# mxngjxa/lshrs

Measured on AMD Instinct MI355X. Metric: vectors/sec hashed (768-d, num_perm=256), higher is better.
Workload: dtype bf16x3 on the matrix cores + f32 replay of the host BLAS inside the proven window (bit-exact f32 sign result)

## Files before the change

### lshrs_amd/csrc/lshrs_common.h

```cpp
#ifndef LSHRS_COMMON_H
#define LSHRS_COMMON_H

#include <hip/hip_runtime.h>
#include <hip/hip_ext.h>
#include <stdint.h>
#include <stddef.h>
#include <math.h>
#include <type_traits>

#include "lshrs_hip.h"

typedef float f32x4 __attribute__((ext_vector_type(4)));
typedef float f32x16 __attribute__((ext_vector_type(16)));
typedef uint32_t u32x2 __attribute__((ext_vector_type(2)));
typedef uint32_t u32x4 __attribute__((ext_vector_type(4)));
typedef __bf16 bf16x8 __attribute__((ext_vector_type(8)));
typedef __bf16 bf16x2 __attribute__((ext_vector_type(2)));
typedef uint16_t u16x8 __attribute__((ext_vector_type(8)));

#define GLOBAL_AS __attribute__((address_space(1)))
#define LDS_AS __attribute__((address_space(3)))
#define LSHRS_HIDDEN __attribute__((visibility("hidden")))

namespace lshrs {
// ... 64 lines not shown
  w.wa = p; w.wb = p + wc; w.wt = p + 2 * wc;
  w.wamax = p + 3 * wc; w.wbmax = w.wamax + cbp; w.wtmax = w.wbmax + cbp; w.wtmax_fine = w.wtmax + cbp;
  return w;
}
struct SigCompact { bool on; int bpb; int ncb; };
inline SigCompact sig_compact(const SigGeom& g, int num_bands, int rows) {
  SigCompact c{false, 0, 0};
  if (g.nt != 8 || rows > 128) return c;
  c.bpb = 256 / rows;
  c.ncb = (num_bands + c.bpb - 1) / c.bpb;
  c.on = c.ncb < g.cb;
  return c;
}
inline int64_t sig_pad4(int64_t v) { return (v + 3) & ~(int64_t)3; }
struct SigCompactWs { float *image, *norms, *norm_max, *wa, *wb, *wamax, *wbmax; int *padcol, *bytetab; };
inline int64_t sig_compact_floats(const SigGeom& g, const SigCompact& c) {
  if (!c.on) return 0;
  return (int64_t)c.ncb * g.ktiles * 8192 + 3 * (int64_t)c.ncb * 256 + 3 * sig_pad4(c.ncb) + (int64_t)c.ncb * 256 * 3;
}
struct SigResident { bool on; int nct; int kt; };
inline SigResident sig_resident(int num_bands, int rows, int dim) {
  SigResident r{false, 0, 0};
  const int64_t real = (int64_t)num_bands * rows;
  if (real > 256 || dim > 256 || dim < 8) return r;
  r.nct = (((int)real + 15) / 16 + 3) / 4 * 4;
  r.kt = dim <= 64 ? 2 : (dim <= 128 ? 4 : 8);
  r.on = r.nct * r.kt <= 64;
  return r;
}
__host__ __device__ inline int res_colmap(int nct, int ct, int m) {
  const int g = m >> 2, e = m & 3, k = ct >> 3;
  const int bits = 4 * (nct - 8 * k < 8 ? nct - 8 * k : 8);
  return 128 * k + bits * g + (bits - 1) - (4 * (ct & 7) + e);
}
inline int64_t sig_resident_floats(const SigResident& r) {
  return r.on ? (int64_t)r.kt * 8192 + 3 * 256 + 3 * 4 + 256 * 3 : 0;
}
inline int64_t sig_workspace_floats(const SigGeom& g, int num_bands, int rows, int dim) {
  return sig_window_offset_floats(g) + sig_window_floats(g) + sig_compact_floats(g, sig_compact(g, num_bands, rows)) +
         sig_resident_floats(sig_resident(num_bands, rows, dim));
}
inline SigCompactWs sig_compact_ws(float* base, const SigGeom& g, const SigCompact& c) {
  SigCompactWs w;
  float* p = base + sig_window_offset_floats(g) + sig_window_floats(g);
  w.image = p; p += (int64_t)c.ncb * g.ktiles * 8192;
  w.norms = p; p += (int64_t)c.ncb * 256;
  w.norm_max = p; p += sig_pad4(c.ncb);
  w.wa = p; p += (int64_t)c.ncb * 256;
  w.wb = p; p += (int64_t)c.ncb * 256;
  w.wamax = p; p += sig_pad4(c.ncb);
  w.wbmax = p; p += sig_pad4(c.ncb);
  w.padcol = reinterpret_cast<int*>(p); p += (int64_t)c.ncb * 256;
  w.bytetab = reinterpret_cast<int*>(p);
  return w;
}
inline SigCompactWs sig_resident_ws(float* base, const SigGeom& g, int num_bands, int rows, const SigResident& r) {
  SigCompactWs w;
  float* p = base + sig_window_offset_floats(g) + sig_window_floats(g) + sig_compact_floats(g, sig_compact(g, num_bands, rows));
  w.image = p; p += (int64_t)r.kt * 8192;
  w.norms = p; p += 256;
  w.norm_max = p; p += 4;
  w.wa = p; p += 256;
  w.wb = p; p += 256;
  w.wamax = p; p += 4;
  w.wbmax = p; p += 4;
  w.padcol = reinterpret_cast<int*>(p); p += 256;
// ... 103 lines not shown
  const float w1 = rem == 1 ? 0.f : (rem == 2 ? v[3] : v[2]);
  const float w2 = rem == 3 ? v[3] : 0.f;
  f32x4 r = part ? f32x4{w0, w1, w2, 0.f} : v;
#pragma unroll
  for (int e = 0; e < 4; ++e) r[e] = gone ? 0.f : r[e];
  return r;
}

__device__ __forceinline__ float row_lanes_sum(const float& v) {
  float s = v + __shfl_xor(v, 16);
  s += __shfl_xor(s, 32);
  return s;
}
__device__ __forceinline__ float row_lanes_max(const float& v) {
  float m = __builtin_fmaxf(v, __shfl_xor(v, 16));
  m = __builtin_fmaxf(m, __shfl_xor(m, 32));
  return m;
}

template <bool RAW_ROOT>
__device__ __forceinline__ float window_root(float v) { return RAW_ROOT ? __builtin_amdgcn_sqrtf(v) : sqrtf(v); }
template <bool RAW_ROOT>
__device__ __forceinline__ float window_hi(float s2, float am, float tau) {
  float window = window_root<RAW_ROOT>(s2) * tau * 1.001f;
  if (am != 0.f && !(am >= 0x1p-32f && am <= 0x1p32f)) window = __builtin_inff();
  return window;
}
template <bool RAW_ROOT>
__device__ __forceinline__ float window_mid(float m2, float tau_b) {
  const float wb = window_root<RAW_ROOT>(m2) * tau_b * 1.001f;
  return wb < __builtin_inff() ? wb : 0.f;
}

constexpr int kEntryColBits = 21;
__host__ __device__ __forceinline__ int64_t flag_entry(int64_t row, int col) { return (row << kEntryColBits) | (int64_t)col; }
__host__ __device__ __forceinline__ int64_t entry_row(int64_t entry) { return entry >> kEntryColBits; }
__host__ __device__ __forceinline__ int entry_col(int64_t entry) { return (int)(entry & ((1 << kEntryColBits) - 1)); }

__device__ __forceinline__ float ykeep(const float& window, const float& y) { return window < __builtin_inff() ? y : __builtin_nanf(""); }

template <bool ALIGNBIT>
__device__ __forceinline__ uint32_t key_byte(uint32_t lo, uint32_t hi, int src, uint32_t mask) {
  const uint32_t v = ALIGNBIT ? __builtin_amdgcn_alignbit(hi, lo, (uint32_t)(src & 31)) : (uint32_t)((((uint64_t)hi << 32) | lo) >> (src & 31));
  return v & mask;
}

struct FixArgs {
  const float* X;
  int64_t ldx;
  int dim;
  int ktiles;
  const float* prow;
  const float* norms;
  const float* tie_coef;
  uint8_t* keys;
  int row_bytes;
  int padcols;
  const int64_t* flag_list;
  const int* flag_count;
  int flag_cap;
  int64_t row_base;
  int64_t* tie_list;
  int tie_cap;
  int* tie_count;
  float tau;
  int blas_model;
// ... 162 lines not shown
```

### lshrs_amd/csrc/sig16.hip

```cpp
#include "lshrs_common.h"

using namespace lshrs;

namespace {
#ifndef LSHRS_X_AUX
#define LSHRS_X_AUX 0
#endif
template <bool COMPACT, bool PARTIAL = false, int W = 8>
__global__ __launch_bounds__(64 * W, 8 / W) void sig16_kernel(const SigArgs args) {
  constexpr int RT = 2;
  constexpr int kRows = 32 * W;
  constexpr int kXDepth = W == 8 ? 3 : 2;
  constexpr int kS1ListCap = W == 8 ? 8192 : 4096;
  constexpr int kWaveRows = 16 * RT;
  constexpr int kPP = 16 / W;
  constexpr int kXPS = RT;
  constexpr int kE = 6 * RT;
  constexpr int kSlices = 12 * RT;
  constexpr int kPHalf = 16 * kFragFloats;
  constexpr int kXTile = kRows * kKTile;
  constexpr int kXWave = kWaveRows * kKTile;
  constexpr int kRingFloats = 3 * kPHalf + kXDepth * kXTile;
  constexpr int kIssues = (kPP + kXPS) / 2;
  constexpr int kIssueStep = kE / kIssues;
  static_assert((kPP + kXPS) % 2 == 0 && kE % kIssues == 0, "DMA issue slots");
  static_assert(3 * kS1ListCap <= kRingFloats, "the epilogue's list stage reuses the ring");
  constexpr int kTabOff = 3 * kS1ListCap;
  constexpr int kWndOff = W == 8 ? kRingFloats : kTabOff + 768 + kRows * 8;
  static_assert(kWndOff + 2 * kRows + 4 <= (W == 8 ? kRingFloats + 512 + 4 : kRingFloats), "windows and counters");
  __shared__ __attribute__((aligned(16))) float lds[W == 8 ? kRingFloats + 512 + 4 : kRingFloats];
  struct Bf16Pairs { bf16x2 p[4]; };

  const int tid = threadIdx.x;
  const int lane = tid & 63;
  const int wave = __builtin_amdgcn_readfirstlane(tid >> 6);
  const int r16 = lane & 15, g = lane >> 4;
  const int ncb = args.ncb;
  const int bid = blockIdx.x;
  const int cb = (bid >> 3) % ncb;
  const int row_tile = ((bid >> 3) / ncb) * 8 + (bid & 7);
  int au_slot = -1, au_rw = -1, au_lane = 0, au_q = 0;
  if (args.audit_list != nullptr) {
    const unsigned u = (unsigned)bid * (unsigned)W + (unsigned)wave;
    if ((int)(u % (unsigned)args.audit_div) == args.audit_phase) {
      const unsigned h = audit_hash(u, args.audit_seed);
      au_slot = (int)(u / (unsigned)args.audit_div);
      au_rw = (int)(h & 15u);
      au_q = (int)((h >> 4) & 7u);
      au_lane = (int)((h >> 7) & 63u);
    }
  }
  if ((int64_t)row_tile * kRows >= args.n) {
    if (au_slot >= 0 && lane == 0) args.audit_list[au_slot] = -1;
    return;
  }
  const int ktiles = args.ktiles;
  const int stages = 2 * ktiles, lasts = stages - 1;
  const char* img = reinterpret_cast<const char*>(args.image) + (size_t)cb * ktiles * 32768;
  const int64_t blk_row0 = (int64_t)row_tile * kRows;
  const int64_t row0 = blk_row0 + wave * kWaveRows;
  const char* xblk = reinterpret_cast<const char*>(args.X + blk_row0 * args.ldx);

  unsigned xfo[2 * RT], xrd[2];
// ... 92 lines not shown
    const int pair = q / 3, step = q % 3, rt = pair >> 2, pr = pair & 3, c = pr >> 1, e = 2 * (pr & 1);
    const float v0 = xr[rt][c][e], v1 = xr[rt][c][e + 1];
    if (step == 0) {
      bf16x2 hp;
      asm("v_cvt_pk_bf16_f32 %0, %1, %2" : "=v"(hp) : "v"(v0), "v"(v1));
      hi[rt].p[pr] = hp;
      r0 = v0 - (float)hp[0];
      r1 = v1 - (float)hp[1];
    } else if (step == 1) {
      bf16x2 mp;
      asm("v_cvt_pk_bf16_f32 %0, %1, %2" : "=v"(mp) : "v"(r0), "v"(r1));
      mid[rt].p[pr] = mp;
    } else {
      ss[rt] = __builtin_amdgcn_fdot2_f32_bf16(hi[rt].p[pr], hi[rt].p[pr], ss[rt], false);
#ifndef LSHRS_AB_NO_XMID_NORM
      sm[rt] = __builtin_amdgcn_fdot2_f32_bf16(mid[rt].p[pr], mid[rt].p[pr], sm[rt], false);
#endif
      asm("v_max3_f32 %0, |%1|, |%2|, %0" : "+v"(amax[rt]) : "v"(v0), "v"(v1));
    }
  };
  auto read_eighth = [&](unsigned base, int e, f32x4 (&f)[2][2]) {
#pragma unroll
    for (int j = 0; j < 2; ++j) {
      f[j][0] = *reinterpret_cast<const LDS_AS f32x4*>(lds_b + (base + (unsigned)(((2 * e + j) * 2 + 0) * 1024)));
      f[j][1] = *reinterpret_cast<const LDS_AS f32x4*>(lds_b + (base + (unsigned)(((2 * e + j) * 2 + 1) * 1024)));
    }
  };
  const unsigned lane16 = (unsigned)lane * 16u;
  auto mfma_one = [&](int ct0, int k, const f32x4 (&f)[2][2], const Bf16Pairs (&hi)[RT], const Bf16Pairs (&mid)[RT], const bool drain = false) {
    const int term = k / (2 * RT), j = (k / RT) % 2, rt = k % RT;
    const bf16x8 a = __builtin_bit_cast(bf16x8, term == 2 ? mid[rt] : hi[rt]);
    const bf16x8 b = __builtin_bit_cast(bf16x8, f[j][term == 1 ? 1 : 0]);
#ifdef LSHRS_T16_BUILTIN
    acc[rt][ct0 + j] = __builtin_amdgcn_mfma_f32_16x16x32_bf16(a, b, acc[rt][ct0 + j], 0, 0, 0);
#else
    if (drain) asm volatile("v_mfma_f32_16x16x32_bf16 %0, %1, %2, %0\n\ts_nop 7\n\ts_nop 4" : "+a"(acc[rt][ct0 + j]) : "v"(a), "v"(b));
    else asm volatile("v_mfma_f32_16x16x32_bf16 %0, %1, %2, %0" : "+a"(acc[rt][ct0 + j]) : "v"(a), "v"(b));
#endif
  };

  f32x4 fa[2][2], fb[2][2];
  Bf16Pairs hs0[RT], ms0[RT], hs1[RT], ms1[RT];

  auto stage = [&](int s, const int ch, const bool first, const Bf16Pairs (&hc)[RT], const Bf16Pairs (&mc)[RT],
                   const Bf16Pairs (&hp)[RT], const Bf16Pairs (&mp)[RT], Bf16Pairs (&hn)[RT], Bf16Pairs (&mn)[RT]) {
    unsigned st = lane16 + fr0;
    asm volatile("" : "+v"(st));
    read_eighth(st, 0, fa);
    __builtin_amdgcn_sched_barrier(0);
#pragma unroll
    for (int k = 0; k < kE; ++k) {
      if (!first) mfma_one(8 * (1 - ch) + 6, k, fb, hp, mp);
      if (ch == 0) {
        if (k % 3 != 2) split_step(2 * kSlices / 3 + (k / 3) * 2 + k % 3, hn, mn);
      }
      __builtin_amdgcn_sched_barrier(0);
    }
    __builtin_amdgcn_s_waitcnt(0xC07F);
    __builtin_amdgcn_sched_barrier(0);
    wait_vmcnt<kXPS>();
    read_eighth(st, 1, fb);
    if (ch == 1) read_x((s >> 1) + 1, xq1);
    __builtin_amdgcn_sched_barrier(0);
#pragma unroll
    for (int k = 0; k < kE; ++k) {
      mfma_one(8 * ch + 0, k, fa, hc, mc);
      __builtin_amdgcn_sched_barrier(0);
    }
    __builtin_amdgcn_s_waitcnt(0xC07F);
    __builtin_amdgcn_sched_barrier(0);
// ... 33 lines not shown
  };
  auto tile = [&](int t, const bool first, Bf16Pairs (&hc)[RT], Bf16Pairs (&mc)[RT], Bf16Pairs (&hp)[RT], Bf16Pairs (&mp)[RT]) {
    stage(2 * t, 0, first, hc, mc, hp, mp, hc, mc);
    stage(2 * t + 1, 1, false, hc, mc, hc, mc, hp, mp);
  };

  auto issue_prologue = [&]() {
    const int t1 = ktiles > 1 ? 1 : 0;
#pragma unroll
    for (int d = 0; d < kPP; ++d) issue_frag(d, 0, fr0);
#pragma unroll
    for (int d = 0; d < kXPS; ++d) { issue_x(d, 0, xq0); issue_x(kXPS + d, 0, xq0); }
#pragma unroll
    for (int d = 0; d < kPP; ++d) issue_frag(d, 1, fr1);
#pragma unroll
    for (int d = 0; d < kXPS; ++d) { issue_x(d, t1, xq1); issue_x(kXPS + d, t1, xq1); }
  };
#ifndef LSHRS_AB_NO_STATIC_PRIO
  if (W == 8 && wave >= 4) __builtin_amdgcn_s_setprio(1);
#endif
  issue_prologue();
  zero_tile_state();
  wait_vmcnt<kPP + 2 * kXPS>();
  __builtin_amdgcn_s_barrier();
  read_x(0, xq0);
#pragma unroll
  for (int q = 0; q < 2 * kSlices / 3; ++q) split_step(q, hs0, ms0);
  tile(0, true, hs0, ms0, hs1, ms1);
  int t = 1;
  for (; t + 1 < ktiles; t += 2) {
    tile(t, false, hs1, ms1, hs0, ms0);
    tile(t + 1, false, hs0, ms0, hs1, ms1);
  }
  if (t < ktiles) {
    tile(t, false, hs1, ms1, hs0, ms0);
#pragma unroll
    for (int k = 0; k < kE; ++k) mfma_one(14, k, fb, hs1, ms1, true);
  } else {
#pragma unroll
    for (int k = 0; k < kE; ++k) mfma_one(14, k, fb, hs0, ms0, true);
  }
  asm volatile("s_waitcnt vmcnt(0)" ::: "memory");
  __builtin_amdgcn_s_barrier();
  asm volatile("s_nop 7\n\ts_nop 7\n\ts_nop 7" ::: "memory");
#pragma unroll
  for (int rt = 0; rt < RT; ++rt)
#pragma unroll
    for (int ct = 0; ct < 16; ++ct) asm volatile("" : "+a"(acc[rt][ct]));

  if (args.clock_probe != nullptr && tid == 0) {
    const unsigned long long slot = (unsigned long long)blockIdx.x;
    args.clock_probe[2 * slot] = __builtin_amdgcn_s_memtime() - t_shader;
    args.clock_probe[2 * slot + 1] = __builtin_amdgcn_s_memrealtime() - t_real;
  }

  int r16e = r16, ge = g, lanee = lane;
  asm volatile("" : "+v"(r16e), "+v"(ge), "+v"(lanee));
  int64_t* l_list = reinterpret_cast<int64_t*>(lds);
  float* l_y = lds + 2 * kS1ListCap;
  int* l_count = reinterpret_cast<int*>(lds + kWndOff + 2 * kRows);
  if (tid == 0) l_count[0] = 0;

  float* wnd_lds = lds + kWndOff + wave * kWaveRows;
  float* wnb_lds = lds + kWndOff + kRows + wave * kWaveRows;
  float* coef_lds = lds + kTabOff;
  static_assert(kTabOff + 512 <= kRingFloats, "coefficients behind the list stage");
#pragma unroll
  for (int i = tid; i < 512; i += 64 * W) coef_lds[i] = i < 256 ? args.wa[cb * 256 + i] : args.wb[cb * 256 + i - 256];
  int* padcol_lds = reinterpret_cast<int*>(lds + kTabOff + 512);
  uint32_t* cw_lds = reinterpret_cast<uint32_t*>(lds + kTabOff + 768);
  static_assert(kTabOff + 768 + kRows * 8 <= kRingFloats, "compact tables behind the coefficients");
  if (COMPACT && tid < 256) padcol_lds[tid] = args.padcol[cb * 256 + tid];
#pragma unroll
  for (int rt = 0; rt < RT; ++rt) {
    const float s2 = row_lanes_sum(ss[rt]), m2 = row_lanes_sum(sm[rt]), am = row_lanes_max(amax[rt]);
    const int64_t myrow = row0 + 16 * rt + r16e;
    if (ge == 0) {
      wnd_lds[16 * rt + r16e] = window_hi<false>(s2, am, args.tau);
      wnb_lds[16 * rt + r16e] = window_mid<false>(m2, args.tau_b);
      if (cb == 0 && args.row_flags != nullptr && myrow < args.n) args.row_flags[myrow] = row_flag_byte(am, s2);
    }
  }
  __builtin_amdgcn_s_waitcnt(0xC07F);
  __builtin_amdgcn_s_barrier();

  const float amax_cb = args.wamax[cb], bmax_cb = args.wbmax[cb];
  {
    uint32_t A[2] = {0u, 0u}, B[2] = {0u, 0u};
#pragma unroll
    for (int rt = 0; rt < 2; ++rt) {
      const f32x4 wnd = *reinterpret_cast<const f32x4*>(wnd_lds + 16 * rt + 4 * ge);
      const f32x4 wnb = *reinterpret_cast<const f32x4*>(wnb_lds + 16 * rt + 4 * ge);
      float tsmax = __builtin_fmaxf(__builtin_fmaxf(wnd[0], wnd[1]), __builtin_fmaxf(wnd[2], wnd[3]));
      if (!(wnd[0] < __builtin_inff()) || !(wnd[1] < __builtin_inff()) || !(wnd[2] < __builtin_inff()) ||
          !(wnd[3] < __builtin_inff()))
        tsmax = __builtin_inff();
      tsmax = tsmax * amax_cb +
              __builtin_fmaxf(__builtin_fmaxf(wnb[0], wnb[1]), __builtin_fmaxf(wnb[2], wnb[3])) * bmax_cb;
      tsmax = tsmax > 0.f ? tsmax : -1.f;
#pragma unroll
      for (int w = 0; w < 8; ++w) {
        float m = __builtin_inff();
#pragma unroll
        for (int reg = 0; reg < 4; ++reg) {
          const float y0 = acc[rt][2 * w][reg], y1 = acc[rt][2 * w + 1][reg];
          const int p0 = 8 * rt + reg * 2;
#ifdef LSHRS_AB_CHEAP_SIGNS
          A[w & 1] = __builtin_amdgcn_alignbit(A[w & 1], __float_as_uint(y0), 31u);
          B[w & 1] = __builtin_amdgcn_alignbit(B[w & 1], __float_as_uint(y1), 31u);
#else
          deposit_positive(A[w & 1], y0, 4 * p0 + (w >> 1), 4 * (p0 + 1) + (w >> 1));
          deposit_positive(B[w & 1], y1, 4 * p0 + (w >> 1), 4 * (p0 + 1) + (w >> 1));
#endif
          asm("v_min3_f32 %0, |%1|, |%2|, %0" : "+v"(m) : "v"(y0), "v"(y1));
        }
        const bool aud = au_rw == 8 * rt + w;
        if (__builtin_amdgcn_ballot_w64(!(m > tsmax)) != 0 || aud) {
          unsigned hits = 0u;
          float ys[8], thrs[8];
#pragma unroll
          for (int half = 0; half < 2; ++half) {
            const int ct = 2 * w + half;
            const float pa = coef_lds[16 * ct + r16e], pb = coef_lds[256 + 16 * ct + r16e];
#pragma unroll
            for (int reg = 0; reg < 4; ++reg) {
              float thr = wnd[reg] * pa + wnb[reg] * pb;
              thr = thr > 0.f ? thr : -1.f;
              ys[4 * half + reg] = acc[rt][ct][reg];
              thrs[4 * half + reg] = thr;
              hits |= (!(__builtin_fabsf(ys[4 * half + reg]) > thr) ? 1u : 0u) << (4 * half + reg);
            }
          }
          if (aud && lanee == au_lane) {
            float yq = ys[0], tq = thrs[0];
#pragma unroll
            for (int q = 1; q < 8; ++q) {
              yq = au_q == q ? ys[q] : yq;
              tq = au_q == q ? thrs[q] : tq;
            }
            const int64_t grow = row0 + 16 * rt + 4 * ge + (au_q & 3);
            const int ct = 2 * w + (au_q >> 2);
            const int colid = COMPACT ? padcol_lds[16 * ct + r16e] : cb * 256 + 16 * ct + r16e;
            const bool keep = ((hits >> au_q) & 1u) == 0u && grow < args.n && colid >= 0 && colid < args.row_bytes * 8 &&
                              tq < __builtin_inff();
            if (args.col_cap > 0) {
              if (keep) {
                const int slot = atomicAdd(args.col_count + colid, 1);
                if (slot < args.col_cap) {
                  const size_t at = (size_t)colid * args.col_cap + slot;
                  args.tie_list[at] = flag_entry(grow, colid) | kAuditBit;
                  args.flag_y[at] = yq;
                  args.flag_thr[at] = tq;
                }
              }
            } else {
              args.audit_list[au_slot] = keep ? flag_entry(grow, colid) : (int64_t)-1;
              args.audit_vals[2 * au_slot] = yq;
              args.audit_vals[2 * au_slot + 1] = tq;
            }
          }
          if (hits != 0u) {
#pragma unroll
            for (int q = 0; q < 8; ++q) {
              const int reg = q & 3, ct = 2 * w + (q >> 2);
              const int64_t grow = row0 + 16 * rt + 4 * ge + reg;
              const int colid = COMPACT ? padcol_lds[16 * ct + r16e] : cb * 256 + 16 * ct + r16e;
              if (((hits >> q) & 1u) != 0u && grow < args.n && (!COMPACT || colid >= 0) &&
                  (args.col_cap == 0 || colid < args.row_bytes * 8)) {
                const int64_t entry = flag_entry(grow, colid);
                const float yk = ykeep(wnd[reg], ys[q]);
                const int pos = atomicAdd(l_count, 1);
                if (pos < kS1ListCap) {
                  l_list[pos] = entry;
                  l_y[pos] = yk;
                } else if (args.col_cap > 0) {
                  atomicAdd(args.tie_count, 1);
                  const int slot = atomicAdd(args.col_count + colid, 1);
                  if (slot < args.col_cap) {
                    args.tie_list[(size_t)colid * args.col_cap + slot] = entry;
                    args.flag_y[(size_t)colid * args.col_cap + slot] = yk;
                  }
                } else {
                  const int slot = atomicAdd(args.tie_count, 1);
                  if (slot < args.tie_cap) {
                    args.tie_list[slot] = entry;
                    if (args.flag_y != nullptr) args.flag_y[slot] = yk;
                  }
                }
              }
            }
          }
        }
      }
    }
    const int pr = lanee >> 2, wq = 2 * (lanee & 3);
    const int rlo = 16 * (pr >> 3) + 8 * (pr & 1) + ((pr >> 1) & 3);
    const uint32_t wlo[2] = {(A[0] & 0xFFFFu) | (B[0] << 16), (A[1] & 0xFFFFu) | (B[1] << 16)};
    const uint32_t whi[2] = {(A[0] >> 16) | (B[0] & 0xFFFF0000u), (A[1] >> 16) | (B[1] & 0xFFFF0000u)};
    const int byte0 = (cb * 8 + wq) * 4;
#pragma unroll
    for (int hl = 0; hl < 2; ++hl) {
      const int64_t grow = row0 + rlo + 4 * hl;
      if (COMPACT) {
        uint32_t* dstw = cw_lds + (wave * kWaveRows + rlo + 4 * hl) * 8 + wq;
        dstw[0] = hl ? whi[0] : wlo[0];
        dstw[1] = hl ? whi[1] : wlo[1];
      } else if (grow < args.n) {
        uint8_t* dst = args.keys + grow * (int64_t)args.row_bytes + byte0;
        const uint32_t w0 = hl ? whi[0] : wlo[0], w1 = hl ? whi[1] : wlo[1];
        if (args.vec_store && byte0 + 8 <= args.row_bytes) {
          *reinterpret_cast<u32x2*>(dst) = u32x2{w0, w1};
        } else {
#pragma unroll
          for (int bsel = 0; bsel < 4; ++bsel) {
            if (byte0 + bsel < args.row_bytes) dst[bsel] = (uint8_t)(w0 >> (8 * bsel));
            if (byte0 + 4 + bsel < args.row_bytes) dst[4 + bsel] = (uint8_t)(w1 >> (8 * bsel));
          }
        }
      }
    }
  }

  __syncthreads();
  if (COMPACT) {
    const int bands_here = args.num_bands - cb * args.bpb < args.bpb ? args.num_bands - cb * args.bpb : args.bpb;
    const int nby = bands_here * args.band_bytes;
    const int byte_base = cb * args.bpb * args.band_bytes;
    const int* tab = args.bytetab + cb * 512;
    for (int idx = tid; idx < kRows * nby; idx += 64 * W) {
      const int rl = idx / nby, o = idx - rl * nby;
      const int64_t grow = blk_row0 + rl;
      if (grow < args.n) {
        const int src = tab[2 * o], w = src >> 5;
        const uint32_t lo = cw_lds[rl * 8 + w], hi = cw_lds[rl * 8 + (w < 7 ? w + 1 : 7)];
        args.keys[grow * (int64_t)args.row_bytes + byte_base + o] = (uint8_t)key_byte<false>(lo, hi, src, (uint32_t)tab[2 * o + 1]);
      }
    }
  }
  const int staged = l_count[0] < kS1ListCap ? l_count[0] : kS1ListCap;
  if (staged > 0 && args.col_cap > 0) {
    if (tid == 0) atomicAdd(args.tie_count, staged);
    for (int e = tid; e < staged; e += 64 * W) {
// ... 4 lines not shown
        args.tie_list[(size_t)col * args.col_cap + slot] = entry;
        args.flag_y[(size_t)col * args.col_cap + slot] = l_y[e];
      }
    }
  } else if (staged > 0) {
    if (tid == 0) l_count[1] = atomicAdd(args.tie_count, staged);
    __syncthreads();
    const int base = l_count[1];
    for (int e = tid; e < staged; e += 64 * W) {
      const int slot = base + e;
      if (slot < args.tie_cap) {
        args.tie_list[slot] = l_list[e];
        if (args.flag_y != nullptr) args.flag_y[slot] = l_y[e];
      }
    }
  }
  if (args.clock_probe != nullptr && tid == 0) {
    const unsigned long long slot = (unsigned long long)gridDim.x + (unsigned long long)blockIdx.x;
    args.clock_probe[2 * slot] = __builtin_amdgcn_s_memtime() - t_shader;
    args.clock_probe[2 * slot + 1] = __builtin_amdgcn_s_memrealtime() - t_real;
  }
}

}

uint32_t lshrs_flags_sig16(void) {
  uint32_t f = 0;
#ifdef LSHRS_AB_NO_XMID_NORM
  f |= LSHRS_BUILD_WRONG_KEYS | (1u << 11);
#endif
#ifdef LSHRS_AB_NO_STATIC_PRIO
  f |= LSHRS_BUILD_TUNED | (1u << 16);
#endif
#ifdef LSHRS_AB_CHEAP_SIGNS
  f |= LSHRS_BUILD_WRONG_KEYS | (1u << 22);
#endif
#ifdef LSHRS_T16_BUILTIN
  f |= LSHRS_BUILD_TUNED | (1u << 20);
#endif
#if LSHRS_X_AUX != 0
  f |= LSHRS_BUILD_TUNED | (1u << 21);
#endif
  return f;
}

int lshrs_launch_sig16(const SigArgs& a, unsigned grid, bool compact, bool partial, bool half, hipStream_t s, hipEvent_t start,
                       hipEvent_t stop) {
  const dim3 g(grid, 1, 1), b(half ? 256 : 512, 1, 1);
  dispatch_bool(half, [&](auto h) {
    dispatch_bool(compact, [&](auto c) {
      dispatch_bool(partial, [&](auto p) {
        hipExtLaunchKernelGGL((sig16_kernel<decltype(c)::value, decltype(p)::value, decltype(h)::value ? 4 : 8>), g, b, 0, s, start, stop, 0, a);
      });
    });
  });
  return -(int)hipGetLastError();
}
```

### lshrs_amd/csrc/sig16r.hip

```cpp
#include "lshrs_common.h"

using namespace lshrs;

namespace {

template <int NCT, int KT>
__global__ __launch_bounds__(64 * res_waves(NCT, KT), 1) void sig16r_kernel(const SigArgs args) {
  constexpr int RT = res_rt(NCT, KT), NW = NCT / 2, kRows = 16 * RT, kResWaves = res_waves(NCT, KT), kResGroups = (NCT + 7) / 8;
  constexpr int kImgFloats = KT * NCT * 512;
  constexpr int kResWaveFloats = res_wave_floats(RT);
  __shared__ __attribute__((aligned(16))) float lds[res_lds_floats<NCT, KT>()];
  struct Bf16Pairs { bf16x2 p[4]; };

  const int tid = threadIdx.x;
  const int lane = tid & 63;
  const int wave = __builtin_amdgcn_readfirstlane(tid >> 6);
  const int r16 = lane & 15, g = lane >> 4;
  float* coef_lds = lds + kImgFloats;
  int* padcol_lds = reinterpret_cast<int*>(lds + kImgFloats + 512);
  int* tab_lds = reinterpret_cast<int*>(lds + kImgFloats + 768);
  float* mine = lds + kImgFloats + 1280 + wave * kResWaveFloats;
  uint32_t* cw_lds = reinterpret_cast<uint32_t*>(mine + 2 * kRows);
  int64_t* l_list = reinterpret_cast<int64_t*>(mine + 11 * kRows);
  float* l_y = mine + 11 * kRows + 2 * kResListCap;
// ... 138 lines not shown
      }
    }

#endif
#ifndef LSHRS_AB_RES_NO_PRIO
    __builtin_amdgcn_s_setprio(0);
#endif
#ifdef LSHRS_AB_RES_PROBE
    asm volatile("" ::: "memory");
    const unsigned long long pr_t1 = __builtin_amdgcn_s_memtime();
#endif
#ifdef LSHRS_AB_RES_NO_EPILOGUE
    {
      float keep = 0.f;
#pragma unroll
      for (int rt = 0; rt < RT; ++rt)
#pragma unroll
        for (int ct = 0; ct < NCT; ++ct) keep += acc[rt][ct][0] + acc[rt][ct][1] + acc[rt][ct][2] + acc[rt][ct][3];
      keep += ss[0] + sm[0] + amax[0];
      if (keep == 123.456f) args.keys[lane] = 1;
    }
    continue;
#endif
    float wnd[RT], wnb[RT], tsmax[RT];
    bool zrow[RT];
#pragma unroll
    for (int rt = 0; rt < RT; ++rt) {
      const float s2 = row_lanes_sum(ss[rt]), m2 = row_lanes_sum(sm[rt]), am = row_lanes_max(amax[rt]);
      const int64_t myrow = row0 + 16 * rt + r16;
      const float window = window_hi<true>(s2, am, args.tau), wb_ = window_mid<true>(m2, args.tau_b);
      if (g == 0 && args.row_flags != nullptr && myrow < args.n) args.row_flags[myrow] = row_flag_byte(am, s2);
      wnd[rt] = window;
      wnb[rt] = wb_;
      float ts = window < __builtin_inff() ? window * amax_cb + wb_ * bmax_cb : __builtin_inff();
      tsmax[rt] = ts > 0.f ? ts : -1.f;
      zrow[rt] = am == 0.f;
    }

    int au_slot = -1, au_rw = -1, au_lane = 0, au_q = 0;
    if (args.audit_list != nullptr && (int)(tile % args.audit_div) == args.audit_phase) {
      const unsigned h = audit_hash((unsigned)tile, args.audit_seed);
      au_slot = (int)(tile / args.audit_div);
      au_rw = (int)((h & 1u) % (unsigned)RT) * 8 + (int)(((h >> 1) & 7u) % (unsigned)NW);
      au_q = (int)((h >> 4) & 7u);
      au_lane = (int)((h >> 7) & 63u);
    }

    {
#pragma unroll
      for (int rt = 0; rt < RT; ++rt) {
        uint32_t word[kResGroups] = {};
#pragma unroll
        for (int w = 0; w < NW; ++w) {
          float m = __builtin_inff();
#pragma unroll
          for (int reg = 0; reg < 4; reg += 2) {
            const float y0 = acc[rt][2 * w][reg], y1 = acc[rt][2 * w][reg + 1];
            word[w >> 2] = __builtin_amdgcn_alignbit(word[w >> 2], __float_as_uint(y0), 31u);
            word[w >> 2] = __builtin_amdgcn_alignbit(word[w >> 2], __float_as_uint(y1), 31u);
            asm("v_min3_f32 %0, |%1|, |%2|, %0" : "+v"(m) : "v"(y0), "v"(y1));
          }
#pragma unroll
          for (int reg = 0; reg < 4; reg += 2) {
            const float y0 = acc[rt][2 * w + 1][reg], y1 = acc[rt][2 * w + 1][reg + 1];
            word[w >> 2] = __builtin_amdgcn_alignbit(word[w >> 2], __float_as_uint(y0), 31u);
            word[w >> 2] = __builtin_amdgcn_alignbit(word[w >> 2], __float_as_uint(y1), 31u);
            asm("v_min3_f32 %0, |%1|, |%2|, %0" : "+v"(m) : "v"(y0), "v"(y1));
          }
          const bool aud = au_rw == 8 * rt + w;
          if (__builtin_amdgcn_ballot_w64(!(m > tsmax[rt])) != 0 || aud) {
            unsigned hits = 0u;
            float ys[8], thrs[8];
#pragma unroll
            for (int half = 0; half < 2; ++half) {
              const int ct = 2 * w + half;
              const f32x4 pa = *reinterpret_cast<const f32x4*>(coef_lds + 16 * ct + 4 * g);
              const f32x4 pb = *reinterpret_cast<const f32x4*>(coef_lds + 256 + 16 * ct + 4 * g);
#pragma unroll
              for (int reg = 0; reg < 4; ++reg) {
                float thr = wnd[rt] * pa[reg] + wnb[rt] * pb[reg];
                thr = thr > 0.f ? thr : -1.f;
                ys[4 * half + reg] = acc[rt][ct][reg];
                thrs[4 * half + reg] = thr;
                hits |= (!(__builtin_fabsf(ys[4 * half + reg]) > thr) ? 1u : 0u) << (4 * half + reg);
              }
            }
            const int64_t grow = row0 + 16 * rt + r16;
            if (aud && lane == au_lane) {
              float yq = ys[0], tq = thrs[0];
#pragma unroll
              for (int q = 1; q < 8; ++q) {
                yq = au_q == q ? ys[q] : yq;
                tq = au_q == q ? thrs[q] : tq;
              }
              const int colid = padcol_lds[16 * (2 * w + (au_q >> 2)) + 4 * g + (au_q & 3)];
              const bool keep = ((hits >> au_q) & 1u) == 0u && grow < args.n && colid >= 0 && tq < __builtin_inff();
              args.audit_list[au_slot] = keep ? flag_entry(grow, colid) : (int64_t)-1;
              args.audit_vals[2 * au_slot] = yq;
              args.audit_vals[2 * au_slot + 1] = tq;
// ... 161 lines not shown
```

### lshrs_amd/csrc/sig_setup.hip

```cpp
#include "lshrs_common.h"

using namespace lshrs;

namespace {

__global__ void pack_image_kernel(const float* __restrict__ P, int num_bands, int rows, int dim, int bb, int nt,
                                  int ktiles, int64_t chunks, f32x4* __restrict__ image) {
  const int64_t c = (int64_t)blockIdx.x * blockDim.x + threadIdx.x;
  if (c >= chunks) return;
  const int lane = (int)(c & 63);
  const int q = (int)((c >> 6) & 3);
  int64_t t = c >> 8;
  const int jt = (int)(t % nt);
  t /= nt;
  const int kt = (int)(t % ktiles);
  const int cb = (int)(t / ktiles);
  const int col = (cb * nt + jt) * 32 + (lane & 31);
  const int band = col / (bb * 8);
  const int bit = col % (bb * 8);
  const int k0 = kt * kKTile + 16 * (lane >> 5) + 4 * q;
  f32x4 v = {0.f, 0.f, 0.f, 0.f};
  if (band < num_bands && bit < rows) {
    const float* src = P + ((int64_t)band * rows + bit) * dim;
#pragma unroll
// ... 62 lines not shown
                                      int* __restrict__ bytetab, int res_nct = 0) {
  const int i = blockIdx.x * blockDim.x + threadIdx.x;
  if (i >= ncb * 256) return;
  const int blk = i >> 8;
  int cc = i & 255;
  {
    const int pc = res_nct > 0 ? ((cc >> 4) < res_nct ? res_colmap(res_nct, cc >> 4, cc & 15) : 256) : cc;
    const int band = blk * bpb + pc / rows, bit = pc % rows;
    padcol[i] = (pc < bpb * rows && band < num_bands) ? band * bb * 8 + bit : -1;
  }
  const int bl = cc / bb, q = cc % bb;
  const bool live = bl < bpb && blk * bpb + bl < num_bands && 8 * q < rows;
  const int nbits = live ? (rows - 8 * q < 8 ? rows - 8 * q : 8) : 0;
  bytetab[2 * i] = live ? bl * rows + 8 * q : 0;
  bytetab[2 * i + 1] = (1 << nbits) - 1;
}

__global__ void compact_gather_kernel(const float* __restrict__ src, const int* __restrict__ padcol, int n,
                                      float* __restrict__ dst) {
  const int i = blockIdx.x * blockDim.x + threadIdx.x;
  if (i < n) dst[i] = padcol[i] >= 0 ? src[padcol[i]] : 0.f;
}

__global__ void pack_image_bf16_t16_kernel(const float* __restrict__ P, int num_bands, int rows, int dim, int bb,
                                           int ktiles, int64_t chunks, u16x8* __restrict__ image, int bpb = 0, int res_nct = 0) {
  const int64_t c = (int64_t)blockIdx.x * blockDim.x + threadIdx.x;
  if (c >= chunks) return;
  const int lane = (int)(c & 63);
  const int part = (int)((c >> 6) & 1);
  const int ct = (int)((c >> 7) & 15);
  const int64_t t = c >> 11;
  const int kt = (int)(t % ktiles);
  const int cb = (int)(t / ktiles);
  const int col = cb * 256 + ct * 16 + (lane & 15);
  int band = col / (bb * 8);
  int bit = col % (bb * 8);
  if (bpb > 0) {
    int cc = col & 255;
    if (res_nct > 0) cc = ct < res_nct ? res_colmap(res_nct, ct, lane & 15) : 256;
    band = cc < bpb * rows ? cb * bpb + cc / rows : num_bands;
    bit = cc % rows;
  }
  const int k0 = kt * kKTile + 8 * (lane >> 4);
  u16x8 v = {0, 0, 0, 0, 0, 0, 0, 0};
  if (band < num_bands && bit < rows) {
    const float* src = P + ((int64_t)band * rows + bit) * dim;
#pragma unroll
    for (int j = 0; j < 8; ++j) {
      if (k0 + j < dim) {
        const float x = src[k0 + j];
        const uint16_t hi = bf16_rne_bits(x);
        const float hif = __uint_as_float((uint32_t)hi << 16);
        v[j] = part == 0 ? hi : bf16_rne_bits(x - hif);
      }
    }
  }
  image[c] = v;
}

}

extern "C" {

int64_t lshrs_sig_workspace_bytes(int32_t num_bands, int32_t rows_per_band, int32_t dim) {
  if (!sig_shape_ok(num_bands, rows_per_band, dim)) return LSHRS_E_BADARG;
  const SigGeom g = sig_geom(num_bands, rows_per_band, dim);
  return sig_workspace_floats(g, num_bands, rows_per_band, dim) * (int64_t)sizeof(float);
// ... 137 lines not shown
```

Measured before the change: 849.3 million.

## Transpose MFMA operands and permute image columns so signs pack directly in registers

Swaps the A/B operands of the bf16 MFMA so each lane holds a row rather than a column, and permutes the packed projection image columns (t16_colmap) so sign bits can be shifted straight into output words with alignbit. This removes the LDS round trip for per-row windows, the deposit_positive bit scatter and the A/B word shuffling. Per-row screen thresholds now come from registers, and a live-column mask built from the norms replaces the old explicit sign deposit. It also shrinks the shared-memory footprint. The risk is wrong keys if the column permutation, live mask or zero-row handling does not exactly match the old bit layout.

```diff
diff --git a/lshrs_amd/csrc/lshrs_common.h b/lshrs_amd/csrc/lshrs_common.h
--- a/lshrs_amd/csrc/lshrs_common.h
+++ b/lshrs_amd/csrc/lshrs_common.h
@@ -120,6 +120,10 @@
   const int g = m >> 2, e = m & 3, k = ct >> 3;
   const int bits = 4 * (nct - 8 * k < 8 ? nct - 8 * k : 8);
   return 128 * k + bits * g + (bits - 1) - (4 * (ct & 7) + e);
+}
+__host__ __device__ inline int t16_colmap(int ct, int m) {
+  const int g = m >> 2, e = m & 3;
+  return 64 * g + 32 * (ct >> 3) + 31 - (4 * (ct & 7) + e);
 }
 inline int64_t sig_resident_floats(const SigResident& r) {
   return r.on ? (int64_t)r.kt * 8192 + 3 * 256 + 3 * 4 + 256 * 3 : 0;
@@ -289,6 +293,14 @@
   return wb < __builtin_inff() ? wb : 0.f;
 }
 
+__device__ __forceinline__ float row_screen(const float& window, const float& wb, const float& amax_cb, const float& bmax_cb) {
+  const float ts = window < __builtin_inff() ? window * amax_cb + wb * bmax_cb : __builtin_inff();
+  return ts > 0.f ? ts : -1.f;
+}
+__device__ __forceinline__ uint32_t shift_sign_in(uint32_t word, const float& y) {
+  return __builtin_amdgcn_alignbit(word, __float_as_uint(y), 31u);
+}
+
 constexpr int kEntryColBits = 21;
 __host__ __device__ __forceinline__ int64_t flag_entry(int64_t row, int col) { return (row << kEntryColBits) | (int64_t)col; }
 __host__ __device__ __forceinline__ int64_t entry_row(int64_t entry) { return entry >> kEntryColBits; }
diff --git a/lshrs_amd/csrc/sig16.hip b/lshrs_amd/csrc/sig16.hip
--- a/lshrs_amd/csrc/sig16.hip
+++ b/lshrs_amd/csrc/sig16.hip
@@ -26,9 +26,9 @@
   static_assert((kPP + kXPS) % 2 == 0 && kE % kIssues == 0, "DMA issue slots");
   static_assert(3 * kS1ListCap <= kRingFloats, "the epilogue's list stage reuses the ring");
   constexpr int kTabOff = 3 * kS1ListCap;
-  constexpr int kWndOff = W == 8 ? kRingFloats : kTabOff + 768 + kRows * 8;
-  static_assert(kWndOff + 2 * kRows + 4 <= (W == 8 ? kRingFloats + 512 + 4 : kRingFloats), "windows and counters");
-  __shared__ __attribute__((aligned(16))) float lds[W == 8 ? kRingFloats + 512 + 4 : kRingFloats];
+  constexpr int kCntOff = W == 8 ? kRingFloats : kTabOff + 768 + kRows * 8;
+  static_assert(kCntOff + 4 <= (W == 8 ? kRingFloats + 4 : kRingFloats), "list counters");
+  __shared__ __attribute__((aligned(16))) float lds[W == 8 ? kRingFloats + 4 : kRingFloats];
   struct Bf16Pairs { bf16x2 p[4]; };
 
   const int tid = threadIdx.x;
@@ -187,10 +187,10 @@
     const bf16x8 a = __builtin_bit_cast(bf16x8, term == 2 ? mid[rt] : hi[rt]);
     const bf16x8 b = __builtin_bit_cast(bf16x8, f[j][term == 1 ? 1 : 0]);
 #ifdef LSHRS_T16_BUILTIN
-    acc[rt][ct0 + j] = __builtin_amdgcn_mfma_f32_16x16x32_bf16(a, b, acc[rt][ct0 + j], 0, 0, 0);
+    acc[rt][ct0 + j] = __builtin_amdgcn_mfma_f32_16x16x32_bf16(b, a, acc[rt][ct0 + j], 0, 0, 0);
 #else
-    if (drain) asm volatile("v_mfma_f32_16x16x32_bf16 %0, %1, %2, %0\n\ts_nop 7\n\ts_nop 4" : "+a"(acc[rt][ct0 + j]) : "v"(a), "v"(b));
-    else asm volatile("v_mfma_f32_16x16x32_bf16 %0, %1, %2, %0" : "+a"(acc[rt][ct0 + j]) : "v"(a), "v"(b));
+    if (drain) asm volatile("v_mfma_f32_16x16x32_bf16 %0, %2, %1, %0\n\ts_nop 7\n\ts_nop 4" : "+a"(acc[rt][ct0 + j]) : "v"(a), "v"(b));
+    else asm volatile("v_mfma_f32_16x16x32_bf16 %0, %2, %1, %0" : "+a"(acc[rt][ct0 + j]) : "v"(a), "v"(b));
 #endif
   };
 
@@ -290,14 +290,17 @@
     tile(t, false, hs1, ms1, hs0, ms0);
     tile(t + 1, false, hs0, ms0, hs1, ms1);
   }
+  Bf16Pairs hd[RT], md[RT];
   if (t < ktiles) {
     tile(t, false, hs1, ms1, hs0, ms0);
 #pragma unroll
-    for (int k = 0; k < kE; ++k) mfma_one(14, k, fb, hs1, ms1, true);
+    for (int rt = 0; rt < RT; ++rt) { hd[rt] = hs1[rt]; md[rt] = ms1[rt]; }
   } else {
 #pragma unroll
-    for (int k = 0; k < kE; ++k) mfma_one(14, k, fb, hs0, ms0, true);
-  }
+    for (int rt = 0; rt < RT; ++rt) { hd[rt] = hs0[rt]; md[rt] = ms0[rt]; }
+  }
+#pragma unroll
+  for (int k = 0; k < kE; ++k) mfma_one(14, k, fb, hd, md, true);
   asm volatile("s_waitcnt vmcnt(0)" ::: "memory");
   __builtin_amdgcn_s_barrier();
   asm volatile("s_nop 7\n\ts_nop 7\n\ts_nop 7" ::: "memory");
@@ -316,134 +319,131 @@
   asm volatile("" : "+v"(r16e), "+v"(ge), "+v"(lanee));
   int64_t* l_list = reinterpret_cast<int64_t*>(lds);
   float* l_y = lds + 2 * kS1ListCap;
-  int* l_count = reinterpret_cast<int*>(lds + kWndOff + 2 * kRows);
+  int* l_count = reinterpret_cast<int*>(lds + kCntOff);
   if (tid == 0) l_count[0] = 0;
 
-  float* wnd_lds = lds + kWndOff + wave * kWaveRows;
-  float* wnb_lds = lds + kWndOff + kRows + wave * kWaveRows;
   float* coef_lds = lds + kTabOff;
   static_assert(kTabOff + 512 <= kRingFloats, "coefficients behind the list stage");
 #pragma unroll
-  for (int i = tid; i < 512; i += 64 * W) coef_lds[i] = i < 256 ? args.wa[cb * 256 + i] : args.wb[cb * 256 + i - 256];
+  for (int i = tid; i < 512; i += 64 * W) {
+    const int src = cb * 256 + t16_colmap((i & 255) >> 4, i & 15);
+    coef_lds[i] = i < 256 ? args.wa[src] : args.wb[src];
+  }
   int* padcol_lds = reinterpret_cast<int*>(lds + kTabOff + 512);
+  uint32_t* live_lds = reinterpret_cast<uint32_t*>(lds + kTabOff + 512);
   uint32_t* cw_lds = reinterpret_cast<uint32_t*>(lds + kTabOff + 768);
   static_assert(kTabOff + 768 + kRows * 8 <= kRingFloats, "compact tables behind the coefficients");
-  if (COMPACT && tid < 256) padcol_lds[tid] = args.padcol[cb * 256 + tid];
+  if (tid < 256) {
+    if (COMPACT) {
+      padcol_lds[tid] = args.padcol[cb * 256 + t16_colmap(tid >> 4, tid & 15)];
+    } else {
+      const unsigned long long live = __builtin_amdgcn_ballot_w64(args.norms[cb * 256 + tid] > 0.f);
+      if (lane == 0) *reinterpret_cast<u32x2*>(live_lds + 2 * wave) = u32x2{(uint32_t)live, (uint32_t)(live >> 32)};
+    }
+  }
+
+  const float amax_cb = args.wamax[cb], bmax_cb = args.wbmax[cb];
+  float wnd[RT], wnb[RT], tsmax[RT];
+  bool zrow[RT];
 #pragma unroll
   for (int rt = 0; rt < RT; ++rt) {
     const float s2 = row_lanes_sum(ss[rt]), m2 = row_lanes_sum(sm[rt]), am = row_lanes_max(amax[rt]);
     const int64_t myrow = row0 + 16 * rt + r16e;
-    if (ge == 0) {
-      wnd_lds[16 * rt + r16e] = window_hi<false>(s2, am, args.tau);
-      wnb_lds[16 * rt + r16e] = window_mid<false>(m2, args.tau_b);
-      if (cb == 0 && args.row_flags != nullptr && myrow < args.n) args.row_flags[myrow] = row_flag_byte(am, s2);
-    }
+    wnd[rt] = window_hi<false>(s2, am, args.tau);
+    wnb[rt] = window_mid<false>(m2, args.tau_b);
+    tsmax[rt] = row_screen(wnd[rt], wnb[rt], amax_cb, bmax_cb);
+    zrow[rt] = am == 0.f;
+    if (ge == 0 && cb == 0 && args.row_flags != nullptr && myrow < args.n) args.row_flags[myrow] = row_flag_byte(am, s2);
   }
   __builtin_amdgcn_s_waitcnt(0xC07F);
   __builtin_amdgcn_s_barrier();
 
-  const float amax_cb = args.wamax[cb], bmax_cb = args.wbmax[cb];
-  {
-    uint32_t A[2] = {0u, 0u}, B[2] = {0u, 0u};
-#pragma unroll
-    for (int rt = 0; rt < 2; ++rt) {
-      const f32x4 wnd = *reinterpret_cast<const f32x4*>(wnd_lds + 16 * rt + 4 * ge);
-      const f32x4 wnb = *reinterpret_cast<const f32x4*>(wnb_lds + 16 * rt + 4 * ge);
-      float tsmax = __builtin_fmaxf(__builtin_fmaxf(wnd[0], wnd[1]), __builtin_fmaxf(wnd[2], wnd[3]));
-      if (!(wnd[0] < __builtin_inff()) || !(wnd[1] < __builtin_inff()) || !(wnd[2] < __builtin_inff()) ||
-          !(wnd[3] < __builtin_inff()))
-        tsmax = __builtin_inff();
-      tsmax = tsmax * amax_cb +
-              __builtin_fmaxf(__builtin_fmaxf(wnb[0], wnb[1]), __builtin_fmaxf(wnb[2], wnb[3])) * bmax_cb;
-      tsmax = tsmax > 0.f ? tsmax : -1.f;
-#pragma unroll
-      for (int w = 0; w < 8; ++w) {
-        float m = __builtin_inff();
-#pragma unroll
-        for (int reg = 0; reg < 4; ++reg) {
-          const float y0 = acc[rt][2 * w][reg], y1 = acc[rt][2 * w + 1][reg];
-          const int p0 = 8 * rt + reg * 2;
-#ifdef LSHRS_AB_CHEAP_SIGNS
-          A[w & 1] = __builtin_amdgcn_alignbit(A[w & 1], __float_as_uint(y0), 31u);
-          B[w & 1] = __builtin_amdgcn_alignbit(B[w & 1], __float_as_uint(y1), 31u);
-#else
-          deposit_positive(A[w & 1], y0, 4 * p0 + (w >> 1), 4 * (p0 + 1) + (w >> 1));
-          deposit_positive(B[w & 1], y1, 4 * p0 + (w >> 1), 4 * (p0 + 1) + (w >> 1));
-#endif
+#pragma unroll
+  for (int rt = 0; rt < RT; ++rt) {
+    const int64_t grow = row0 + 16 * rt + r16e;
+    uint32_t word[2] = {0u, 0u};
+#pragma unroll
+    for (int w = 0; w < 8; ++w) {
+      float m = __builtin_inff();
+#pragma unroll
+      for (int half = 0; half < 2; ++half)
+#pragma unroll
+        for (int reg = 0; reg < 4; reg += 2) {
+          const float y0 = acc[rt][2 * w + half][reg], y1 = acc[rt][2 * w + half][reg + 1];
+          word[w >> 2] = shift_sign_in(word[w >> 2], y0);
+          word[w >> 2] = shift_sign_in(word[w >> 2], y1);
           asm("v_min3_f32 %0, |%1|, |%2|, %0" : "+v"(m) : "v"(y0), "v"(y1));
         }
-        const bool aud = au_rw == 8 * rt + w;
-        if (__builtin_amdgcn_ballot_w64(!(m > tsmax)) != 0 || aud) {
-          unsigned hits = 0u;
-          float ys[8], thrs[8];
-#pragma unroll
-          for (int half = 0; half < 2; ++half) {
-            const int ct = 2 * w + half;
-            const float pa = coef_lds[16 * ct + r16e], pb = coef_lds[256 + 16 * ct + r16e];
-#pragma unroll
-            for (int reg = 0; reg < 4; ++reg) {
-              float thr = wnd[reg] * pa + wnb[reg] * pb;
-              thr = thr > 0.f ? thr : -1.f;
-              ys[4 * half + reg] = acc[rt][ct][reg];
-              thrs[4 * half + reg] = thr;
-              hits |= (!(__builtin_fabsf(ys[4 * half + reg]) > thr) ? 1u : 0u) << (4 * half + reg);
+      const bool aud = au_rw == 8 * rt + w;
+      if (__builtin_amdgcn_ballot_w64(!(m > tsmax[rt])) != 0 || aud) {
+        unsigned hits = 0u;
+        float ys[8], thrs[8];
+#pragma unroll
+        for (int half = 0; half < 2; ++half) {
+          const int ct = 2 * w + half;
+          const f32x4 pa = *reinterpret_cast<const f32x4*>(coef_lds + 16 * ct + 4 * ge);
+          const f32x4 pb = *reinterpret_cast<const f32x4*>(coef_lds + 256 + 16 * ct + 4 * ge);
+#pragma unroll
+          for (int reg = 0; reg < 4; ++reg) {
+            float thr = wnd[rt] * pa[reg] + wnb[rt] * pb[reg];
+            thr = thr > 0.f ? thr : -1.f;
+            ys[4 * half + reg] = acc[rt][ct][reg];
+            thrs[4 * half + reg] = thr;
+            hits |= (!(__builtin_fabsf(ys[4 * half + reg]) > thr) ? 1u : 0u) << (4 * half + reg);
+          }
+        }
+        if (aud && lanee == au_lane) {
+          float yq = ys[0], tq = thrs[0];
+#pragma unroll
+          for (int q = 1; q < 8; ++q) {
+            yq = au_q == q ? ys[q] : yq;
+            tq = au_q == q ? thrs[q] : tq;
+          }
+          const int ct = 2 * w + (au_q >> 2), mpos = 4 * ge + (au_q & 3);
+          const int colid = COMPACT ? padcol_lds[16 * ct + mpos] : cb * 256 + t16_colmap(ct, mpos);
+          const bool keep = ((hits >> au_q) & 1u) == 0u && grow < args.n && colid >= 0 && colid < args.row_bytes * 8 &&
+                            tq < __builtin_inff();
+          if (args.col_cap > 0) {
+            if (keep) {
+              const int slot = atomicAdd(args.col_count + colid, 1);
+              if (slot < args.col_cap) {
+                const size_t at = (size_t)colid * args.col_cap + slot;
+                args.tie_list[at] = flag_entry(grow, colid) | kAuditBit;
+                args.flag_y[at] = yq;
+                args.flag_thr[at] = tq;
+              }
             }
+          } else {
+            args.audit_list[au_slot] = keep ? flag_entry(grow, colid) : (int64_t)-1;
+            args.audit_vals[2 * au_slot] = yq;
+            args.audit_vals[2 * au_slot + 1] = tq;
           }
-          if (aud && lanee == au_lane) {
-            float yq = ys[0], tq = thrs[0];
-#pragma unroll
-            for (int q = 1; q < 8; ++q) {
-              yq = au_q == q ? ys[q] : yq;
-              tq = au_q == q ? thrs[q] : tq;
-            }
-            const int64_t grow = row0 + 16 * rt + 4 * ge + (au_q & 3);
-            const int ct = 2 * w + (au_q >> 2);
-            const int colid = COMPACT ? padcol_lds[16 * ct + r16e] : cb * 256 + 16 * ct + r16e;
-            const bool keep = ((hits >> au_q) & 1u) == 0u && grow < args.n && colid >= 0 && colid < args.row_bytes * 8 &&
-                              tq < __builtin_inff();
-            if (args.col_cap > 0) {
-              if (keep) {
+        }
+        if (hits != 0u) {
+#pragma unroll
+          for (int q = 0; q < 8; ++q) {
+            const int reg = q & 3, ct = 2 * w + (q >> 2);
+            const int colid = COMPACT ? padcol_lds[16 * ct + 4 * ge + reg] : cb * 256 + t16_colmap(ct, 4 * ge + reg);
+            if (((hits >> q) & 1u) != 0u && grow < args.n && (!COMPACT || colid >= 0) &&
+                (args.col_cap == 0 || colid < args.row_bytes * 8)) {
+              const int64_t entry = flag_entry(grow, colid);
+              const float yk = ykeep(wnd[rt], ys[q]);
+              const int pos = atomicAdd(l_count, 1);
+              if (pos < kS1ListCap) {
+                l_list[pos] = entry;
+                l_y[pos] = yk;
+              } else if (args.col_cap > 0) {
+                atomicAdd(args.tie_count, 1);
                 const int slot = atomicAdd(args.col_count + colid, 1);
                 if (slot < args.col_cap) {
-                  const size_t at = (size_t)colid * args.col_cap + slot;
-                  args.tie_list[at] = flag_entry(grow, colid) | kAuditBit;
-                  args.flag_y[at] = yq;
-                  args.flag_thr[at] = tq;
+                  args.tie_list[(size_t)colid * args.col_cap + slot] = entry;
+                  args.flag_y[(size_t)colid * args.col_cap + slot] = yk;
                 }
-              }
-            } else {
-              args.audit_list[au_slot] = keep ? flag_entry(grow, colid) : (int64_t)-1;
-              args.audit_vals[2 * au_slot] = yq;
-              args.audit_vals[2 * au_slot + 1] = tq;
-            }
-          }
-          if (hits != 0u) {
-#pragma unroll
-            for (int q = 0; q < 8; ++q) {
-              const int reg = q & 3, ct = 2 * w + (q >> 2);
-              const int64_t grow = row0 + 16 * rt + 4 * ge + reg;
-              const int colid = COMPACT ? padcol_lds[16 * ct + r16e] : cb * 256 + 16 * ct + r16e;
-              if (((hits >> q) & 1u) != 0u && grow < args.n && (!COMPACT || colid >= 0) &&
-                  (args.col_cap == 0 || colid < args.row_bytes * 8)) {
-                const int64_t entry = flag_entry(grow, colid);
-                const float yk = ykeep(wnd[reg], ys[q]);
-                const int pos = atomicAdd(l_count, 1);
-                if (pos < kS1ListCap) {
-                  l_list[pos] = entry;
-                  l_y[pos] = yk;
-                } else if (args.col_cap > 0) {
-                  atomicAdd(args.tie_count, 1);
-                  const int slot = atomicAdd(args.col_count + colid, 1);
-                  if (slot < args.col_cap) {
-                    args.tie_list[(size_t)colid * args.col_cap + slot] = entry;
-                    args.flag_y[(size_t)colid * args.col_cap + slot] = yk;
-                  }
-                } else {
-                  const int slot = atomicAdd(args.tie_count, 1);
-                  if (slot < args.tie_cap) {
-                    args.tie_list[slot] = entry;
-                    if (args.flag_y != nullptr) args.flag_y[slot] = yk;
-                  }
+              } else {
+                const int slot = atomicAdd(args.tie_count, 1);
+                if (slot < args.tie_cap) {
+                  args.tie_list[slot] = entry;
+                  if (args.flag_y != nullptr) args.flag_y[slot] = yk;
                 }
               }
             }
@@ -451,21 +451,16 @@
         }
       }
     }
-    const int pr = lanee >> 2, wq = 2 * (lanee & 3);
-    const int rlo = 16 * (pr >> 3) + 8 * (pr & 1) + ((pr >> 1) & 3);
-    const uint32_t wlo[2] = {(A[0] & 0xFFFFu) | (B[0] << 16), (A[1] & 0xFFFFu) | (B[1] << 16)};
-    const uint32_t whi[2] = {(A[0] >> 16) | (B[0] & 0xFFFF0000u), (A[1] >> 16) | (B[1] & 0xFFFF0000u)};
-    const int byte0 = (cb * 8 + wq) * 4;
-#pragma unroll
-    for (int hl = 0; hl < 2; ++hl) {
-      const int64_t grow = row0 + rlo + 4 * hl;
-      if (COMPACT) {
-        uint32_t* dstw = cw_lds + (wave * kWaveRows + rlo + 4 * hl) * 8 + wq;
-        dstw[0] = hl ? whi[0] : wlo[0];
-        dstw[1] = hl ? whi[1] : wlo[1];
-      } else if (grow < args.n) {
+    uint32_t w0 = zrow[rt] ? 0u : ~word[0], w1 = zrow[rt] ? 0u : ~word[1];
+    const int byte0 = (cb * 8 + 2 * ge) * 4;
+    if (COMPACT) {
+      *reinterpret_cast<u32x2*>(cw_lds + (wave * kWaveRows + 16 * rt + r16e) * 8 + 2 * ge) = u32x2{w0, w1};
+    } else {
+      const u32x2 live = *reinterpret_cast<const u32x2*>(live_lds + 2 * ge);
+      w0 &= live[0];
+      w1 &= live[1];
+      if (grow < args.n) {
         uint8_t* dst = args.keys + grow * (int64_t)args.row_bytes + byte0;
-        const uint32_t w0 = hl ? whi[0] : wlo[0], w1 = hl ? whi[1] : wlo[1];
         if (args.vec_store && byte0 + 8 <= args.row_bytes) {
           *reinterpret_cast<u32x2*>(dst) = u32x2{w0, w1};
         } else {
@@ -536,9 +531,6 @@
 #ifdef LSHRS_AB_NO_STATIC_PRIO
   f |= LSHRS_BUILD_TUNED | (1u << 16);
 #endif
-#ifdef LSHRS_AB_CHEAP_SIGNS
-  f |= LSHRS_BUILD_WRONG_KEYS | (1u << 22);
-#endif
 #ifdef LSHRS_T16_BUILTIN
   f |= LSHRS_BUILD_TUNED | (1u << 20);
 #endif
diff --git a/lshrs_amd/csrc/sig16r.hip b/lshrs_amd/csrc/sig16r.hip
--- a/lshrs_amd/csrc/sig16r.hip
+++ b/lshrs_amd/csrc/sig16r.hip
@@ -194,8 +194,7 @@
       if (g == 0 && args.row_flags != nullptr && myrow < args.n) args.row_flags[myrow] = row_flag_byte(am, s2);
       wnd[rt] = window;
       wnb[rt] = wb_;
-      float ts = window < __builtin_inff() ? window * amax_cb + wb_ * bmax_cb : __builtin_inff();
-      tsmax[rt] = ts > 0.f ? ts : -1.f;
+      tsmax[rt] = row_screen(window, wb_, amax_cb, bmax_cb);
       zrow[rt] = am == 0.f;
     }
 
@@ -218,15 +217,15 @@
 #pragma unroll
           for (int reg = 0; reg < 4; reg += 2) {
             const float y0 = acc[rt][2 * w][reg], y1 = acc[rt][2 * w][reg + 1];
-            word[w >> 2] = __builtin_amdgcn_alignbit(word[w >> 2], __float_as_uint(y0), 31u);
-            word[w >> 2] = __builtin_amdgcn_alignbit(word[w >> 2], __float_as_uint(y1), 31u);
+            word[w >> 2] = shift_sign_in(word[w >> 2], y0);
+            word[w >> 2] = shift_sign_in(word[w >> 2], y1);
             asm("v_min3_f32 %0, |%1|, |%2|, %0" : "+v"(m) : "v"(y0), "v"(y1));
           }
 #pragma unroll
           for (int reg = 0; reg < 4; reg += 2) {
             const float y0 = acc[rt][2 * w + 1][reg], y1 = acc[rt][2 * w + 1][reg + 1];
-            word[w >> 2] = __builtin_amdgcn_alignbit(word[w >> 2], __float_as_uint(y0), 31u);
-            word[w >> 2] = __builtin_amdgcn_alignbit(word[w >> 2], __float_as_uint(y1), 31u);
+            word[w >> 2] = shift_sign_in(word[w >> 2], y0);
+            word[w >> 2] = shift_sign_in(word[w >> 2], y1);
             asm("v_min3_f32 %0, |%1|, |%2|, %0" : "+v"(m) : "v"(y0), "v"(y1));
           }
           const bool aud = au_rw == 8 * rt + w;
diff --git a/lshrs_amd/csrc/sig_setup.hip b/lshrs_amd/csrc/sig_setup.hip
--- a/lshrs_amd/csrc/sig_setup.hip
+++ b/lshrs_amd/csrc/sig_setup.hip
@@ -118,7 +118,7 @@
   const int64_t t = c >> 11;
   const int kt = (int)(t % ktiles);
   const int cb = (int)(t / ktiles);
-  const int col = cb * 256 + ct * 16 + (lane & 15);
+  const int col = cb * 256 + t16_colmap(ct, lane & 15);
   int band = col / (bb * 8);
   int bit = col % (bb * 8);
   if (bpb > 0) {
```

Result: faster. 858.1 million (median of 6 runs) (+1.0%).
